# wangyunpeng139/3_ORB_SLAM3_SelfNote

Measured on AMD Instinct MI355X. Metric: frames/sec ORB extract+match, 752x480, higher is better.
Workload: dtype u8; 1 GPU; BASELINE configs[2]: extract + SearchByProjection match, 1000x1000 candidates, synthetic frame stream; image=752x480, nfeatures=1000, nlevels=8, batch=256, distinct_frames_per_gpu=2048, streams=4

## Files before the change

3_orb_slam3_selfnote_amd/csrc/orb_fast_score.h:

```cpp
#pragma once
#include <hip/hip_runtime.h>
#include <stdint.h>
#include "orb_common.h"

typedef short pk16 __attribute__((ext_vector_type(2)));

__host__ __device__ __forceinline__ int fast_score_S(const uint8_t *c ) {
  constexpr int Pt = FAST_TILE_PITCH;
  const int v = c[0];
  const pk16 V2 = {(short)v, (short)-v};
  const pk16 K = {(short)-1, (short)1};
  pk16 d[16];
#define ORB_RING(k, off) { const short cc = (short)c[off]; const pk16 C = {cc, cc}; d[k] = C * K + V2; }
  ORB_RING(0, 3 * Pt + 0)   ORB_RING(1, 3 * Pt + 1)   ORB_RING(2, 2 * Pt + 2)    ORB_RING(3, 1 * Pt + 3)
  ORB_RING(4, 3)            ORB_RING(5, -1 * Pt + 3)  ORB_RING(6, -2 * Pt + 2)   ORB_RING(7, -3 * Pt + 1)
  ORB_RING(8, -3 * Pt)      ORB_RING(9, -3 * Pt - 1)  ORB_RING(10, -2 * Pt - 2)  ORB_RING(11, -1 * Pt - 3)
  ORB_RING(12, -3)          ORB_RING(13, 1 * Pt - 3)  ORB_RING(14, 2 * Pt - 2)   ORB_RING(15, 3 * Pt - 1)
#undef ORB_RING
  pk16 m2[8], m4[8];
#pragma unroll
  for (int i = 0; i < 8; i++) m2[i] = __builtin_elementwise_min(d[2 * i + 1], d[(2 * i + 2) & 15]);
#pragma unroll
  for (int i = 0; i < 8; i++) m4[i] = __builtin_elementwise_min(m2[i], m2[(i + 1) & 7]);
  pk16 A;
#pragma unroll
  for (int i = 0; i < 8; i++) {
    const pk16 m8 = __builtin_elementwise_min(m4[i], m4[(i + 2) & 7]);
    const pk16 e = __builtin_elementwise_max(d[2 * i], d[(2 * i + 9) & 15]);
    const pk16 p = __builtin_elementwise_min(m8, e);
    A = i == 0 ? p : __builtin_elementwise_max(A, p);
  }
  const int a = A.x, b = A.y;
  const int S = a > b ? a : b;
  return S < 0 ? 0 : (S > 255 ? 255 : S);
}
```

3_orb_slam3_selfnote_amd/csrc/orb_kernels.h:

```cpp
#pragma once
#include <hip/hip_runtime.h>
#include <type_traits>
#include "orb_common.h"
#include "orb_fast_score.h"
#include "orb_sincos.h"

#define WAVE 64

__constant__ __attribute__((aligned(16))) int8_t c_pattern[1024] = {
#include "../../include/orb_pattern_data.inc"
};

struct DiscTab { uint32_t w[64][6]; };
constexpr DiscTab make_disc_tab() {
  DiscTab t{};
  const int umax[16] = {15, 15, 15, 15, 14, 14, 14, 13, 13, 12, 11, 10, 9, 8, 6, 3};
  int n = 0;
  for (int v = -15; v <= 15; v++) {
    const int d = umax[v < 0 ? -v : v];
    for (int u = -d; u <= d; u++) {
      const int lane = n & 63, k = n >> 6;
      t.w[lane][k >> 2] |= (uint32_t)(uint8_t)(int8_t)u << (8 * (k & 3));
      t.w[lane][3 + (k >> 2)] |= (uint32_t)(uint8_t)(int8_t)v << (8 * (k & 3));
      n++;
    }
  }
  return t;
}
__constant__ __attribute__((aligned(16))) DiscTab c_disc = make_disc_tab();

__device__ __forceinline__ int reflect101(int p, int n) {
  if (n == 1) return 0;
  while (p < 0 || p >= n) p = p < 0 ? -p : 2 * (n - 1) - p;
  return p;
}

__device__ __forceinline__ const uint8_t *level_plane(const FrameParams &P, int frame, int level, int &pitch) {
  if (level == 0) {
    pitch = (int)P.img0_stride;
    return P.img0 + (size_t)frame * P.img0_frame_stride;
  }
  pitch = P.geom[level].pitch;
  return P.pyr + (size_t)frame * P.pyr_fs + P.geom[level].off;
}

__device__ __forceinline__ void xcd_map(int nitems, uint32_t magic, int nframes, int &frame, int &item) {
  const unsigned b = blockIdx.x;
  const unsigned full = (unsigned)(nframes & ~7);
  const unsigned nfull = full * (unsigned)nitems;
  const bool inFull = b < nfull;
  const unsigned q = inFull ? (b >> 3) : (b - nfull);
  unsigned g = __umulhi(q, magic);
  unsigned r = q - g * (unsigned)nitems;
  if (r >= (unsigned)nitems) { g++; r -= (unsigned)nitems; }
  frame = (int)(inFull ? (b & 7u) + 8u * g : full + g);
  item = (int)r;
}

template <int CTRL, int ROWMASK>
__device__ __forceinline__ int dpp_or_zero(int v) { return __builtin_amdgcn_update_dpp(0, v, CTRL, ROWMASK, 0xf, false); }
__device__ __forceinline__ uint32_t mul24(uint32_t a, uint32_t u) {
  uint32_t d;
  asm("v_mul_u32_u24 %0, %1, %2" : "=v"(d) : "s"(u), "v"(a));
  return d;
}
__device__ __forceinline__ uint32_t mul24_vv(uint32_t a, uint32_t b) { return __umul24(a, b); }

__device__ __forceinline__ int wave_sum_i32(int v) {
  v += dpp_or_zero<0x111, 0xf>(v);
  v += dpp_or_zero<0x112, 0xf>(v);
  v += dpp_or_zero<0x114, 0xf>(v);
  v += dpp_or_zero<0x118, 0xf>(v);
  v += dpp_or_zero<0x142, 0xa>(v);
  v += dpp_or_zero<0x143, 0xc>(v);
  return __builtin_amdgcn_readlane(v, 63);
}

__device__ __forceinline__ uint32_t wave_incl_scan(uint32_t x) {
  int v = (int)x;
  v += dpp_or_zero<0x111, 0xf>(v);
  v += dpp_or_zero<0x112, 0xf>(v);
  v += dpp_or_zero<0x114, 0xf>(v);
  v += dpp_or_zero<0x118, 0xf>(v);
  v += dpp_or_zero<0x142, 0xa>(v);
  v += dpp_or_zero<0x143, 0xc>(v);
  return (uint32_t)v;
}

template <int NT>
__device__ uint32_t lds_excl_scan(uint32_t *a, int n, uint32_t *sw) {
  const int tid = threadIdx.x, lane = tid & 63, wid = tid >> 6;
  constexpr int NW = NT / 64;
  uint32_t carry = 0;
  for (int base = 0; base < n; base += NT) {
    int i = base + tid;
    uint32_t v = i < n ? a[i] : 0u;
    uint32_t inc = wave_incl_scan(v);
    if (lane == 63) sw[wid] = inc;
    __syncthreads();
    const uint32_t wsum = lane < NW ? sw[lane] : 0u;
    const uint32_t wincl = wave_incl_scan(wsum);
    const int widu = __builtin_amdgcn_readfirstlane(wid);
    const uint32_t woff = (uint32_t)__builtin_amdgcn_readlane((int)(wincl - wsum), widu);
    const uint32_t tot = (uint32_t)__builtin_amdgcn_readlane((int)wincl, NW - 1);
    if (i < n) a[i] = carry + woff + inc - v;
    carry += tot;
    __syncthreads();
  }
  return carry;
}

#define RESIZE_ROWS_MAX 16
#define RESIZE_MAXSRC 32
__global__ __launch_bounds__(256) void k_resize(FrameParams P, int level, int smemRowBytes, int tPitch, int maxSrc) {
  extern __shared__ __align__(16) uint8_t smem_rs[];
  const LevelGeom G = P.geom[level];
  const LevelGeom Gs = P.geom[level - 1];
  const int tid = threadIdx.x;
  int frame, rowTile;
  xcd_map((G.h + G.resizeRows - 1) / G.resizeRows, G.rowTileMagic, P.nframes, frame, rowTile);
  const int dy0 = rowTile * G.resizeRows;
  const int nrows = min(G.resizeRows, G.h - dy0);
  int spitch;
  const uint8_t *src = level_plane(P, frame, level - 1, spitch);
  uint8_t *dstplane = P.pyr + (size_t)frame * P.pyr_fs + G.off;
  const int wq = (G.w + 3) & ~3, qw = wq >> 2;
  __shared__ int2 sY[RESIZE_ROWS_MAX];
  if (tid < nrows) sY[tid] = P.ytab[G.ytabBase + dy0 + tid];

  if (tPitch > 0) {
    const int syFirst = min(max(P.ytab[G.ytabBase + dy0].x, 0), Gs.h - 1);
    const int syLast = min(max(P.ytab[G.ytabBase + dy0 + nrows - 1].x + 1, 0), Gs.h - 1);
    const int nsrc = min(syLast - syFirst + 1, maxSrc);
    uint8_t *sRows = smem_rs;
    uint8_t *sT = sRows + (size_t)maxSrc * smemRowBytes;
    uint4 *sRowRec = reinterpret_cast<uint4 *>(sT + (((size_t)maxSrc * tPitch + 15) & ~(size_t)15));
    const int4 *xtab4 = reinterpret_cast<const int4 *>(P.xtab + G.xtabBase);
    int4 xtPre[2];
#pragma unroll
    for (int k = 0; k < 2; k++) { const int p = tid + 256 * k; xtPre[k] = 2 * p < wq ? xtab4[p] : make_int4(0, 0, 0, 0); }
    const bool aligned = ((((uintptr_t)src) | (uintptr_t)spitch) & 3u) == 0;
    const uint8_t *src0 = src + (size_t)syFirst * spitch;
    if (aligned) {
      const int cpr = smemRowBytes >> 4, nfull = Gs.w >> 4;
      const float inv_cpr = 1.0f / (float)cpr;
      for (int idx = tid; idx < cpr * nsrc; idx += 256) {
        const int r = (int)(((float)idx + 0.5f) * inv_cpr), c = idx - (int)mul24((uint32_t)r, (uint32_t)cpr);
        if (c < nfull)
          __builtin_amdgcn_global_load_lds((const __attribute__((address_space(1))) void *)(src0 + (mul24((uint32_t)r, (uint32_t)spitch) + 16u * (uint32_t)c)),
                                           (__attribute__((address_space(3))) void *)(sRows + (size_t)(idx - (tid & 63)) * 16), 16, 0, 0);
      }
      const int ndw = (Gs.w + 3) >> 2, d0 = 4 * nfull, ntail = ndw - d0;
      const bool lastRowPartial = (Gs.w & 3) != 0;
      for (int idx = tid; idx < ntail * nsrc; idx += 256) {
        const int r = idx / ntail, d = d0 + (idx - r * ntail);
        const uint8_t *rowp = src0 + mul24((uint32_t)r, (uint32_t)spitch);
        uint32_t v;
        if (lastRowPartial && d == ndw - 1 && syFirst + r == Gs.h - 1 && spitch < 4 * ndw) {
          v = 0;
          for (int b = 0; 4 * d + b < Gs.w; b++) v |= (uint32_t)rowp[4 * d + b] << (8 * b);
        } else {
          v = *reinterpret_cast<const uint32_t *>(rowp + 4 * d);
        }
        *reinterpret_cast<uint32_t *>(sRows + mul24((uint32_t)r, (uint32_t)smemRowBytes) + 4 * d) = v;
      }
    } else {
      const float inv_w = 1.0f / (float)Gs.w;
      for (int idx = tid; idx < Gs.w * nsrc; idx += 256) {
        const int r = (int)(((float)idx + 0.5f) * inv_w), c = idx - (int)mul24((uint32_t)r, (uint32_t)Gs.w);
        sRows[mul24((uint32_t)r, (uint32_t)smemRowBytes) + c] = src0[mul24((uint32_t)r, (uint32_t)spitch) + c];
      }
    }
    if (tid < nrows) {
      const int2 yt = P.ytab[G.ytabBase + dy0 + tid];
      const int sy0 = min(max(yt.x, 0), Gs.h - 1), sy1 = min(max(yt.x + 1, 0), Gs.h - 1);
      sRowRec[tid] = make_uint4((uint32_t)((sy0 - syFirst) * tPitch), (uint32_t)((sy1 - syFirst) * tPitch), (uint32_t)yt.y, (uint32_t)((dy0 + tid) * G.pitch));
    }
    __syncthreads();
    typedef unsigned short u16x2 __attribute__((ext_vector_type(2)));
    auto dot2 = [](uint32_t pix, uint32_t coef) -> uint32_t {
      u16x2 x, y;
      __builtin_memcpy(&x, &pix, 4); __builtin_memcpy(&y, &coef, 4);
// ... 934 lines not shown
    for (int t = 0; t < 2; t++) {
      const uint32_t idx = (uint32_t)(lane + 64 * t), r = (idx * 21846u) >> 16, c = idx - 3u * r;
      if (idx < 111u)
        __builtin_amdgcn_global_load_lds((const __attribute__((address_space(1))) void *)(brow + (mul24(r, (uint32_t)G.bpitch) + 16u * c)),
                                         (__attribute__((address_space(3))) void *)&myPatch[idx * 16], 16, 0, 0);
    }
  }
  int m10 = 0, m01 = 0;
  int dv[12], du[12], dval[12];
  {
    const uint32_t uw[3] = {dw0.x, dw0.y, dw0.z}, vw[3] = {dw0.w, dw1.x, dw1.y};
#pragma unroll
    for (int t = 0; t < 12; t++) {
      du[t] = (int)(int8_t)(uw[t >> 2] >> (8 * (t & 3)));
      dv[t] = (int)(int8_t)(vw[t >> 2] >> (8 * (t & 3)));
    }
  }
  __shared__ __align__(16) uint8_t sDisc[4][31 * 48];
  uint8_t *myDisc = sDisc[threadIdx.x >> 6];
  if (((((uintptr_t)img) | (uintptr_t)pitch) & 3u) == 0) {
    const int qx0 = (X - 15) & ~3, qox = (X - 15) - qx0;
    const uint8_t *irow = img + (size_t)(Y - 15) * pitch + qx0;
#pragma unroll
    for (int t = 0; t < 2; t++) {
      const uint32_t idx = (uint32_t)(lane + 64 * t), r = (idx * 21846u) >> 16, c = idx - 3u * r;
      if (idx < 93u)
        __builtin_amdgcn_global_load_lds((const __attribute__((address_space(1))) void *)(irow + (mul24(r, (uint32_t)pitch) + 16u * c)),
                                         (__attribute__((address_space(3))) void *)&myDisc[idx * 16], 16, 0, 0);
    }
    asm volatile("s_waitcnt vmcnt(0)" ::: "memory");
    const uint8_t *dc = myDisc + 15 * 48 + qox + 15;
#pragma unroll
    for (int t = 0; t < 12; t++) dval[t] = dc[dv[t] * 48 + du[t]];
  } else {
#pragma unroll
    for (int t = 0; t < 12; t++) dval[t] = centre[dv[t] * pitch + du[t]];
  }
#pragma unroll
  for (int t = 0; t < 12; t++) { m10 += du[t] * dval[t]; m01 += dv[t] * dval[t]; }
  m10 = wave_sum_i32(m10);
  m01 = wave_sum_i32(m01);
  const float angle = fast_atan2_deg((float)m01, (float)m10);

  const float factorPI = (float)(3.1415926535897932384626433832795 / 180.f);
  const float arad = angle * factorPI;
  const float a = orbsc::ref_cosf(arad), b = orbsc::ref_sinf(arad);
  const uint8_t *bc = myPatch + 18 * 48 + pox + 18;
  constexpr int bp = 48;
  unsigned long long bits[4];
  int o0[4], o1[4];
#pragma unroll
  for (int r = 0; r < 4; r++) {
    const float x0 = (float)(int8_t)(pw[r] & 0xff), y0 = (float)(int8_t)((pw[r] >> 8) & 0xff);
    const float x1 = (float)(int8_t)((pw[r] >> 16) & 0xff), y1 = (float)(int8_t)(pw[r] >> 24);
    o0[r] = __float2int_rn(x0 * b + y0 * a) * bp + __float2int_rn(x0 * a - y0 * b);
    o1[r] = __float2int_rn(x1 * b + y1 * a) * bp + __float2int_rn(x1 * a - y1 * b);
  }
  asm volatile("s_waitcnt vmcnt(0)" ::: "memory");
  int v0[4], v1[4];
#pragma unroll
  for (int r = 0; r < 4; r++) { v0[r] = bc[o0[r]]; v1[r] = bc[o1[r]]; }
#pragma unroll
  for (int r = 0; r < 4; r++) bits[r] = __ballot(v0[r] < v1[r]);
  if (dst < P.cap) {
    uint32_t *dd = reinterpret_cast<uint32_t *>(P.out_desc + ((size_t)frame * P.cap + dst) * 32);
    if (lane < 8) {
      unsigned long long w = bits[lane >> 1];
      dd[lane] = (uint32_t)((lane & 1) ? (w >> 32) : w);
    }
    if (lane == 8) {
      KpOut k;
      k.x = (float)X;
      k.y = (float)Y;
      if (level != 0) { k.x = k.x * G.scale; k.y = k.y * G.scale; }
      k.size = G.kpsize;
      k.angle = angle;
      k.response = (float)(packed >> 24);
      k.octave = level;
      k.class_id = -1;
      reinterpret_cast<KpOut *>(P.out_kps)[(size_t)frame * P.cap + dst] = k;
    }
  }
}

template <int LANEBIT>
__device__ __forceinline__ int tr_step(int a, int b, int lane) {
  constexpr int CTRL = LANEBIT == 3 ? 0x140 : LANEBIT == 2 ? 0x141 : LANEBIT == 1 ? 0x4e : 0xb1;
  const bool hi = ((lane >> LANEBIT) & 1) != 0;
  const int keep = hi ? b : a, give = hi ? a : b;
  return keep + dpp_or_zero<CTRL, 0xf>(give);
}
template <int LOG, int LO, int N, class F>
__device__ __forceinline__ void tr_range(F &one, int lane, int &r10, int &r01) {
  if constexpr (N == 1) one(std::integral_constant<int, LO>{}, r10, r01);
  else {
    int a10, a01, b10, b01;
    tr_range<LOG, LO, N / 2>(one, lane, a10, a01);
    tr_range<LOG, LO + N / 2, N / 2>(one, lane, b10, b01);
    constexpr int S = N == 2 ? 0 : N == 4 ? 1 : N == 8 ? 2 : 3;
    r10 = tr_step<LOG - 1 - S>(a10, b10, lane);
    r01 = tr_step<LOG - 1 - S>(a01, b01, lane);
  }
}

typedef const __attribute__((address_space(3))) uint8_t *LdsBytes;
typedef const __attribute__((address_space(1))) uint8_t *GlobalBytes;
#define DESC_BUF (37 * 48)
#define DESC_WAVE_LDS (2 * DESC_BUF + 512)

template <int K>
__device__ __forceinline__ void describe_block(const FrameParams &P) {
  static_assert(K == 4 || K == 8 || K == 16, "a block is a quad, a half row or a row of DPP lanes");
  constexpr int LOG = K == 16 ? 4 : K == 8 ? 3 : 2;
  const int lane = threadIdx.x & 63;
  const int wid = __builtin_amdgcn_readfirstlane((int)(threadIdx.x >> 6));
  int frame, wg;
  xcd_map(ORB_DESCRIBE_GROUPS(P.totalKp, K), P.magicKpBlk, P.nframes, frame, wg);
  const int j0 = (wg * 4 + wid) * K;
  if (j0 >= P.totalKp) return;
  __shared__ __align__(16) uint8_t sDesc[4][DESC_WAVE_LDS];
  uint8_t *myLds = sDesc[wid];

  int cL = 0, lpL = 0, kbL = 0;
  if (lane < P.nlevels) {
    const int2 v = reinterpret_cast<const int2 *>(P.lcnt + (size_t)frame * P.nlevels * 2)[lane];
    cL = v.x; lpL = v.y;
    kbL = P.geom[lane].kpBase;
  }
  const int j = j0 + lane;
  int level = 0, kb = __builtin_amdgcn_readlane(kbL, 0), myCount = __builtin_amdgcn_readlane(cL, 0);
  int lapBefore = 0, monoBefore = 0, nTot = myCount, lapTot = __builtin_amdgcn_readlane(lpL, 0);
  for (int l = 1; l < P.nlevels; l++) {
    const int c = __builtin_amdgcn_readlane(cL, l), lp = __builtin_amdgcn_readlane(lpL, l), base = __builtin_amdgcn_readlane(kbL, l);
    const bool ge = j >= base;
    level = ge ? l : level; kb = ge ? base : kb; myCount = ge ? c : myCount;
    lapBefore = ge ? lapTot : lapBefore; monoBefore = ge ? nTot - lapTot : monoBefore;
    nTot += c; lapTot += lp;
  }
  if (j0 == 0 && lane == 0) { P.out_counts[frame * 2] = nTot; P.out_counts[frame * 2 + 1] = nTot - lapTot; }
  const bool valid = lane < K && j < P.totalKp && j - kb < myCount;
  const uint32_t validMask = (uint32_t)__ballot(valid);
  if (validMask == 0) return;
  uint32_t packed = 0, rk = 0;
  if (valid) { packed = P.lkp[(size_t)frame * P.lkp_fs + j]; rk = P.lrank[(size_t)frame * P.lkp_fs + j]; }
  const int X = (int)(packed & 0xfff) + ORB_MIN_BORDER, Y = (int)((packed >> 12) & 0xfff) + ORB_MIN_BORDER;
  const int dst = (rk & 0x8000u) ? nTot - 1 - (lapBefore + (int)(rk & 0x7fff)) : monoBefore + (int)(rk & 0x7fff);
  int pitch = (int)P.img0_stride;
  const uint8_t *img = P.img0 + (size_t)frame * P.img0_frame_stride;
  if (level != 0) { pitch = P.geom[level].pitch; img = P.pyr + (size_t)frame * P.pyr_fs + P.geom[level].off; }
  const uint8_t *centre = img + (size_t)Y * pitch + X;
  const uint32_t dmaMask = (uint32_t)__ballot(valid && ((((uintptr_t)img) | (uintptr_t)pitch) & 3u) == 0);
  const uint32_t cenLo = (uint32_t)(uintptr_t)centre, cenHi = (uint32_t)((uintptr_t)centre >> 32);

  const uint4 dw0 = *reinterpret_cast<const uint4 *>(&c_disc.w[lane][0]);
  const uint2 dw1 = *reinterpret_cast<const uint2 *>(&c_disc.w[lane][4]);
  const uint32_t uw[3] = {dw0.x, dw0.y, dw0.z}, vw[3] = {dw0.w, dw1.x, dw1.y};
  uint32_t doff2[6];
#pragma unroll
  for (int t = 0; t < 12; t += 2) {
    auto place = [&](int tt) { return (uint32_t)((int)(int8_t)(vw[tt >> 2] >> (8 * (tt & 3))) * 48 + (int)(int8_t)(uw[tt >> 2] >> (8 * (tt & 3))) + 15 * 48 + 15); };
    doff2[t >> 1] = place(t) | (place(t + 1) << 16);
    asm volatile("" : "+v"(doff2[t >> 1]));
  }
  const uint32_t cr0 = ((uint32_t)lane * 21846u) >> 16, cc0 = 16u * ((uint32_t)lane - 3u * cr0);
  const uint32_t cr1 = ((uint32_t)(lane + 64) * 21846u) >> 16, cc1 = 16u * ((uint32_t)(lane + 64) - 3u * cr1);
  auto issue = [&](const uint8_t *row0, uint32_t rowPitch, int which, uint32_t nchunks) {
    uint8_t *buf = myLds + which * DESC_BUF;
    asm volatile("s_waitcnt lgkmcnt(0)" ::: "memory");
    __builtin_amdgcn_global_load_lds((const __attribute__((address_space(1))) void *)(row0 + (mul24(cr0, rowPitch) + cc0)),
                                     (__attribute__((address_space(3))) void *)&buf[lane * 16], 16, 0, 0);
    if ((uint32_t)lane + 64u < nchunks)
      __builtin_amdgcn_global_load_lds((const __attribute__((address_space(1))) void *)(row0 + (mul24(cr1, rowPitch) + cc1)),
                                       (__attribute__((address_space(3))) void *)&buf[(lane + 64) * 16], 16, 0, 0);
  };
  auto centre_of = [&](uint32_t lo, uint32_t hi, int k) {
    return (uintptr_t)(uint32_t)__builtin_amdgcn_readlane((int)lo, k) | ((uintptr_t)(uint32_t)__builtin_amdgcn_readlane((int)hi, k) << 32);
  };
  auto issue_disc = [&](int k) {
    const uintptr_t c15 = centre_of(cenLo, cenHi, k) - 15;
    const uint32_t p = (uint32_t)__builtin_amdgcn_readlane(pitch, k);
    issue(reinterpret_cast<const uint8_t *>(c15 & ~(uintptr_t)3) - 15 * (size_t)p, p, k & 1, 93u);
  };

  if (dmaMask & 1u) issue_disc(0);
  auto one = [&](auto kc, int &p10, int &p01) {
    constexpr int k = decltype(kc)::value;
    const bool nextDma = k + 1 < K && ((dmaMask >> ((k + 1) & 31)) & 1u) != 0;
    if (nextDma) issue_disc(k + 1);
    p10 = 0; p01 = 0;
    if ((validMask >> k) & 1u) {
      uint32_t dval[12], dpk[3];
      const uintptr_t cen = centre_of(cenLo, cenHi, k);
      if ((dmaMask >> k) & 1u) {
        if (nextDma) asm volatile("s_waitcnt vmcnt(2)" ::: "memory");
        else asm volatile("s_waitcnt vmcnt(0)" ::: "memory");
        const LdsBytes dc = (LdsBytes)(myLds + (k & 1) * DESC_BUF + ((cen - 15) & 3));
#pragma unroll
        for (int t = 0; t < 12; t++) dval[t] = dc[(t & 1) ? doff2[t >> 1] >> 16 : doff2[t >> 1] & 0xffffu];
#pragma unroll
        for (int g = 0; g < 3; g++) dpk[g] = (dval[4 * g] | (dval[4 * g + 1] << 8)) | ((dval[4 * g + 2] | (dval[4 * g + 3] << 8)) << 16);
      } else {
        const GlobalBytes cp = (GlobalBytes)cen;
        const int p = __builtin_amdgcn_readlane(pitch, k);
        uint32_t uo[3], vo[3];
#pragma unroll
        for (int g = 0; g < 3; g++) { uo[g] = uw[g]; vo[g] = vw[g]; asm volatile("" : "+v"(uo[g]), "+v"(vo[g])); }
#pragma unroll
        for (int t = 0; t < 12; t++)
          dval[t] = cp[(int)(int8_t)(vo[t >> 2] >> (8 * (t & 3))) * p + (int)(int8_t)(uo[t >> 2] >> (8 * (t & 3)))];
#pragma unroll
        for (int g = 0; g < 3; g++) dpk[g] = (dval[4 * g] | (dval[4 * g + 1] << 8)) | ((dval[4 * g + 2] | (dval[4 * g + 3] << 8)) << 16);
      }
#pragma unroll
      for (int g = 0; g < 3; g++) {
        const uint32_t d = dpk[g] ^ 0x80808080u;
        p10 = __builtin_amdgcn_sdot4((int)uw[g], (int)d, p10, false);
        p01 = __builtin_amdgcn_sdot4((int)vw[g], (int)d, p01, false);
      }
    }
  };
  int r10, r01;
  tr_range<LOG, 0, K>(one, lane, r10, r01);
  int2 *sRed = reinterpret_cast<int2 *>(myLds + 2 * DESC_BUF);
  sRed[lane] = make_int2(r10, r01);
  int m10 = 0, m01 = 0;
  if (lane < K) {
    const int q = (int)(__builtin_bitreverse32((uint32_t)lane) >> (32 - LOG));
#pragma unroll
    for (int g = 0; g < 64 / K; g++) { const int2 v = sRed[q + K * g]; m10 += v.x; m01 += v.y; }
  }
  const int bpitch = P.geom[level].bpitch;
  const uint8_t *bcentre = P.blur + (size_t)frame * P.blur_fs + P.geom[level].boff + (size_t)Y * bpitch + X;
  const uint32_t bcenLo = (uint32_t)(uintptr_t)bcentre, bcenHi = (uint32_t)((uintptr_t)bcentre >> 32);
  auto issue_patch = [&](int k, int which) {
    const uintptr_t c18 = centre_of(bcenLo, bcenHi, k) - 18;
    const uint32_t p = (uint32_t)__builtin_amdgcn_readlane(bpitch, k);
    issue(reinterpret_cast<const uint8_t *>(c18 & ~(uintptr_t)3) - 18 * (size_t)p, p, which, 111u);
  };
  issue_patch(__builtin_ctz(validMask), 0);

  const float angle = fast_atan2_deg((float)m01, (float)m10);
  const float factorPI = (float)(3.1415926535897932384626433832795 / 180.f);
  const float arad = angle * factorPI;
  const float ca = orbsc::ref_cosf(arad), sb = orbsc::ref_sinf(arad);

  float pf[16];
#pragma unroll
  for (int r = 0; r < 4; r++) {
    const uint32_t pw = reinterpret_cast<const uint32_t *>(c_pattern)[r * 64 + lane];
    pf[4 * r] = (float)(int8_t)(pw & 0xff); pf[4 * r + 1] = (float)(int8_t)((pw >> 8) & 0xff);
    pf[4 * r + 2] = (float)(int8_t)((pw >> 16) & 0xff); pf[4 * r + 3] = (float)(int8_t)(pw >> 24);
  }
  constexpr int bp = 48;
  int which = 0;
  for (uint32_t m = validMask; m != 0; which ^= 1) {
    const int k = __builtin_ctz(m);
    m &= m - 1;
    if (m != 0) issue_patch(__builtin_ctz(m), which ^ 1);
    const float a = __builtin_bit_cast(float, __builtin_amdgcn_readlane(__builtin_bit_cast(int, ca), k));
    const float b = __builtin_bit_cast(float, __builtin_amdgcn_readlane(__builtin_bit_cast(int, sb), k));
    auto rn_bits = [](float v) { return __float_as_uint(v + 12582912.0f); };
    constexpr uint32_t RN_BIAS = 48u * 0x400000u + 0x4b400000u;
    uint32_t o0[4], o1[4];
#pragma unroll
    for (int r = 0; r < 4; r++) {
      const float x0 = pf[4 * r], y0 = pf[4 * r + 1], x1 = pf[4 * r + 2], y1 = pf[4 * r + 3];
      o0[r] = __umul24(rn_bits(x0 * b + y0 * a), (uint32_t)bp) + rn_bits(x0 * a - y0 * b);
      o1[r] = __umul24(rn_bits(x1 * b + y1 * a), (uint32_t)bp) + rn_bits(x1 * a - y1 * b);
    }
    if (m != 0) asm volatile("s_waitcnt vmcnt(2)" ::: "memory");
    else asm volatile("s_waitcnt vmcnt(0)" ::: "memory");
    const uint32_t bc = (uint32_t)(uintptr_t)(LdsBytes)myLds + (uint32_t)(which * DESC_BUF + 18 * 48 + 18) + (uint32_t)((centre_of(bcenLo, bcenHi, k) - 18) & 3) - RN_BIAS;
    int v0[4], v1[4];
#pragma unroll
    for (int r = 0; r < 4; r++) { v0[r] = *(LdsBytes)(uintptr_t)(bc + o0[r]); v1[r] = *(LdsBytes)(uintptr_t)(bc + o1[r]); }
    unsigned long long bits[4];
#pragma unroll
    for (int r = 0; r < 4; r++) bits[r] = __ballot(v0[r] < v1[r]);
    const int d = __builtin_amdgcn_readlane(dst, k);
    if (d < P.cap && lane < 8) {
      const unsigned long long w = bits[lane >> 1];
      reinterpret_cast<uint32_t *>(P.out_desc + ((size_t)frame * P.cap + d) * 32)[lane] = (uint32_t)((lane & 1) ? (w >> 32) : w);
    }
  }
  if (valid && dst < P.cap) {
    KpOut o;
    o.x = (float)X;
    o.y = (float)Y;
    if (level != 0) { const float sc = P.geom[level].scale; o.x = o.x * sc; o.y = o.y * sc; }
    o.size = P.geom[level].kpsize;
    o.angle = angle;
    o.response = (float)(packed >> 24);
    o.octave = level;
    o.class_id = -1;
    reinterpret_cast<KpOut *>(P.out_kps)[(size_t)frame * P.cap + dst] = o;
  }
}

template <int K>
__global__ __launch_bounds__(256, K == 1 ? 1 : 8) void k_describe(FrameParams P) {
  if constexpr (K == 1) describe_one(P);
  else describe_block<K>(P);
}

__global__ __launch_bounds__(256) void k_cvt_gray(const uint8_t *src, int rows, int cols, size_t sstride, int ch, int rgb, uint8_t *dst,
                                                  size_t dstride) {
  const int q = blockIdx.x * 256 + threadIdx.x, y = blockIdx.y;
  const int x0 = 4 * q;
  if (x0 >= cols || y >= rows) return;
  const uint8_t *s = src + (size_t)y * sstride + (size_t)x0 * ch;
  const int cr = rgb ? 0 : 2, cb = rgb ? 2 : 0;
  uint32_t packed = 0;
  const int n = min(4, cols - x0);
  for (int j = 0; j < n; j++) {
    const uint32_t g = ((uint32_t)s[j * ch + cr] * 4899u + (uint32_t)s[j * ch + 1] * 9617u + (uint32_t)s[j * ch + cb] * 1868u + 8192u) >> 14;
    packed |= g << (8 * j);
  }
  uint8_t *d = dst + (size_t)y * dstride + x0;
  if (n == 4 && ((((uintptr_t)dst) | dstride) & 3u) == 0) *reinterpret_cast<uint32_t *>(d) = packed;
  else for (int j = 0; j < n; j++) d[j] = (uint8_t)(packed >> (8 * j));
}

__device__ __forceinline__ uint8_t clahe_lut_entry(int v, int t, int clipLimit, float lutScale, uint32_t *hist, int *part) {
  if (clipLimit > 0) {
    int excess = v > clipLimit ? v - clipLimit : 0;
    if (v > clipLimit) v = clipLimit;
    const int ws = wave_sum_i32(excess);
    if ((t & 63) == 0) part[t >> 6] = ws;
    __syncthreads();
    const int clipped = part[0] + part[1] + part[2] + part[3];
    const int redistBatch = clipped / 256;
    const int residual = clipped - redistBatch * 256;
    v += redistBatch;
    if (residual != 0) {
      const int step = max(256 / residual, 1);
      if (t % step == 0 && t / step < residual) v++;
    }
  }
  __syncthreads();
  hist[t] = (uint32_t)v;
  __syncthreads();
  for (int d = 1; d < 256; d <<= 1) {
    const uint32_t a = t >= d ? hist[t - d] : 0u;
    __syncthreads();
    hist[t] += a;
    __syncthreads();
  }
  const int r = __float2int_rn(__fmul_rn((float)(int)hist[t], lutScale));
  return (uint8_t)min(max(r, 0), 255);
}

__global__ __launch_bounds__(256) void k_clahe_lut(const uint8_t *src, int rows, int cols, size_t sstride, int tilesX, int tw, int th, int clipLimit,
                                                   float lutScale, uint8_t *lut) {
  __shared__ uint32_t hist[256];
  __shared__ int part[4];
  const int t = threadIdx.x, tile = blockIdx.x, tx = tile % tilesX, ty = tile / tilesX;
  hist[t] = 0;
  __syncthreads();
  const int x0 = tx * tw, y0 = ty * th;
  for (int i = t; i < tw * th; i += 256) {
    int y = y0 + i / tw, x = x0 + i % tw;
    if (y >= rows) y = 2 * (rows - 1) - y;
    if (x >= cols) x = 2 * (cols - 1) - x;
    atomicAdd(&hist[src[(size_t)y * sstride + x]], 1u);
  }
  __syncthreads();
  lut[(size_t)tile * 256 + t] = clahe_lut_entry((int)hist[t], t, clipLimit, lutScale, hist, part);
}

__host__ __device__ __forceinline__ void clahe_tile_coord(int v, float inv_t, int ntiles, int &t1, int &t2, float &a, float &a1) {
// ... 257 lines not shown
```

Measured before the change: 296,600 frames/s.

## Use row-major disc layout with vector LDS reads and packed-half min3/max3 FAST score

The orientation moment loop now assigns each lane half of one disc row. It reads 20 contiguous bytes from LDS with a b128 plus b32 load, aligns them with alignbyte, and applies masked u/v weight words. This replaces 12 scattered byte LDS reads per lane. The FAST score biases its values to be positive so packed fp16 minimum/maximum can act as 3-input min/max on the integer bit patterns, and it reduces the final max as a tree to shorten the dependency chain. The change adds one extra sdot group and relies on the fp16 ordering trick, which is only correct while the biased values stay positive.

```diff
diff --git a/3_orb_slam3_selfnote_amd/csrc/orb_fast_score.h b/3_orb_slam3_selfnote_amd/csrc/orb_fast_score.h
--- a/3_orb_slam3_selfnote_amd/csrc/orb_fast_score.h
+++ b/3_orb_slam3_selfnote_amd/csrc/orb_fast_score.h
@@ -5,10 +5,30 @@
 
 typedef short pk16 __attribute__((ext_vector_type(2)));
 
+constexpr int FAST_BIAS = 2048;
+__host__ __device__ __forceinline__ pk16 fast_min3(pk16 a, pk16 b, pk16 c) {
+#if defined(__HIP_DEVICE_COMPILE__)
+  typedef _Float16 pkh __attribute__((ext_vector_type(2)));
+  return __builtin_bit_cast(pk16, __builtin_elementwise_minimum(__builtin_elementwise_minimum(__builtin_bit_cast(pkh, a), __builtin_bit_cast(pkh, b)),
+                                                                __builtin_bit_cast(pkh, c)));
+#else
+  return __builtin_elementwise_min(__builtin_elementwise_min(a, b), c);
+#endif
+}
+__host__ __device__ __forceinline__ pk16 fast_max3(pk16 a, pk16 b, pk16 c) {
+#if defined(__HIP_DEVICE_COMPILE__)
+  typedef _Float16 pkh __attribute__((ext_vector_type(2)));
+  return __builtin_bit_cast(pk16, __builtin_elementwise_maximum(__builtin_elementwise_maximum(__builtin_bit_cast(pkh, a), __builtin_bit_cast(pkh, b)),
+                                                                __builtin_bit_cast(pkh, c)));
+#else
+  return __builtin_elementwise_max(__builtin_elementwise_max(a, b), c);
+#endif
+}
+
 __host__ __device__ __forceinline__ int fast_score_S(const uint8_t *c ) {
   constexpr int Pt = FAST_TILE_PITCH;
   const int v = c[0];
-  const pk16 V2 = {(short)v, (short)-v};
+  const pk16 V2 = {(short)(FAST_BIAS + v), (short)(FAST_BIAS - v)};
   const pk16 K = {(short)-1, (short)1};
   pk16 d[16];
 #define ORB_RING(k, off) { const short cc = (short)c[off]; const pk16 C = {cc, cc}; d[k] = C * K + V2; }
@@ -17,20 +37,18 @@
   ORB_RING(8, -3 * Pt)      ORB_RING(9, -3 * Pt - 1)  ORB_RING(10, -2 * Pt - 2)  ORB_RING(11, -1 * Pt - 3)
   ORB_RING(12, -3)          ORB_RING(13, 1 * Pt - 3)  ORB_RING(14, 2 * Pt - 2)   ORB_RING(15, 3 * Pt - 1)
 #undef ORB_RING
-  pk16 m2[8], m4[8];
+  pk16 m2[8], m4[8], p[8];
 #pragma unroll
   for (int i = 0; i < 8; i++) m2[i] = __builtin_elementwise_min(d[2 * i + 1], d[(2 * i + 2) & 15]);
 #pragma unroll
   for (int i = 0; i < 8; i++) m4[i] = __builtin_elementwise_min(m2[i], m2[(i + 1) & 7]);
-  pk16 A;
 #pragma unroll
   for (int i = 0; i < 8; i++) {
-    const pk16 m8 = __builtin_elementwise_min(m4[i], m4[(i + 2) & 7]);
     const pk16 e = __builtin_elementwise_max(d[2 * i], d[(2 * i + 9) & 15]);
-    const pk16 p = __builtin_elementwise_min(m8, e);
-    A = i == 0 ? p : __builtin_elementwise_max(A, p);
+    p[i] = fast_min3(m4[i], m4[(i + 2) & 7], e);
   }
-  const int a = A.x, b = A.y;
+  const pk16 A = __builtin_elementwise_max(fast_max3(p[0], p[1], p[2]), fast_max3(fast_max3(p[3], p[4], p[5]), p[6], p[7]));
+  const int a = A.x - FAST_BIAS, b = A.y - FAST_BIAS;
   const int S = a > b ? a : b;
   return S < 0 ? 0 : (S > 255 ? 255 : S);
 }
diff --git a/3_orb_slam3_selfnote_amd/csrc/orb_kernels.h b/3_orb_slam3_selfnote_amd/csrc/orb_kernels.h
--- a/3_orb_slam3_selfnote_amd/csrc/orb_kernels.h
+++ b/3_orb_slam3_selfnote_amd/csrc/orb_kernels.h
@@ -12,12 +12,12 @@
 };
 
 struct DiscTab { uint32_t w[64][6]; };
+constexpr int kDiscUmax[16] = {15, 15, 15, 15, 14, 14, 14, 13, 13, 12, 11, 10, 9, 8, 6, 3};
 constexpr DiscTab make_disc_tab() {
   DiscTab t{};
-  const int umax[16] = {15, 15, 15, 15, 14, 14, 14, 13, 13, 12, 11, 10, 9, 8, 6, 3};
   int n = 0;
   for (int v = -15; v <= 15; v++) {
-    const int d = umax[v < 0 ? -v : v];
+    const int d = kDiscUmax[v < 0 ? -v : v];
     for (int u = -d; u <= d; u++) {
       const int lane = n & 63, k = n >> 6;
       t.w[lane][k >> 2] |= (uint32_t)(uint8_t)(int8_t)u << (8 * (k & 3));
@@ -28,6 +28,11 @@
   return t;
 }
 __constant__ __attribute__((aligned(16))) DiscTab c_disc = make_disc_tab();
+constexpr uint64_t make_disc_umax_nibbles() {
+  uint64_t p = 0;
+  for (int v = 0; v < 16; v++) p |= (uint64_t)kDiscUmax[v] << (4 * v);
+  return p;
+}
 
 __device__ __forceinline__ int reflect101(int p, int n) {
   if (n == 1) return 0;
@@ -1268,15 +1273,22 @@
   const uint32_t dmaMask = (uint32_t)__ballot(valid && ((((uintptr_t)img) | (uintptr_t)pitch) & 3u) == 0);
   const uint32_t cenLo = (uint32_t)(uintptr_t)centre, cenHi = (uint32_t)((uintptr_t)centre >> 32);
 
-  const uint4 dw0 = *reinterpret_cast<const uint4 *>(&c_disc.w[lane][0]);
-  const uint2 dw1 = *reinterpret_cast<const uint2 *>(&c_disc.w[lane][4]);
-  const uint32_t uw[3] = {dw0.x, dw0.y, dw0.z}, vw[3] = {dw0.w, dw1.x, dw1.y};
-  uint32_t doff2[6];
-#pragma unroll
-  for (int t = 0; t < 12; t += 2) {
-    auto place = [&](int tt) { return (uint32_t)((int)(int8_t)(vw[tt >> 2] >> (8 * (tt & 3))) * 48 + (int)(int8_t)(uw[tt >> 2] >> (8 * (tt & 3))) + 15 * 48 + 15); };
-    doff2[t >> 1] = place(t) | (place(t + 1) << 16);
-    asm volatile("" : "+v"(doff2[t >> 1]));
+  const int drow = min(lane >> 1, 30), dhalf = lane & 1, dvv = drow - 15;
+  const uint32_t rowOff = (uint32_t)(drow * 48 + 16 * dhalf);
+  uint32_t wu[4], wv[4];
+  {
+    const int d = (int)((make_disc_umax_nibbles() >> (4 * (dvv < 0 ? -dvv : dvv))) & 15u);
+    const int first = dhalf ? 0 : 15 - d, end = lane < 62 ? (dhalf ? d : 16) : first;
+    const uint32_t vrep = (uint32_t)(dvv & 0xff) * 0x01010101u;
+#pragma unroll
+    for (int i = 0; i < 4; i++) {
+      const int lo = min(max(first - 4 * i, 0), 4), hi = min(max(end - 4 * i, 0), 4);
+      const uint32_t inside = (uint32_t)(0xffffffffull << (8 * lo)) & ~(uint32_t)(0xffffffffull << (8 * hi));
+      auto ub = [](int u0) { return (uint32_t)(uint8_t)u0 | ((uint32_t)(uint8_t)(u0 + 1) << 8) | ((uint32_t)(uint8_t)(u0 + 2) << 16) | ((uint32_t)(uint8_t)(u0 + 3) << 24); };
+      wu[i] = (dhalf ? ub(4 * i + 1) : ub(4 * i - 15)) & inside;
+      wv[i] = vrep & inside;
+      asm volatile("" : "+v"(wu[i]), "+v"(wv[i]));
+    }
   }
   const uint32_t cr0 = ((uint32_t)lane * 21846u) >> 16, cc0 = 16u * ((uint32_t)lane - 3u * cr0);
   const uint32_t cr1 = ((uint32_t)(lane + 64) * 21846u) >> 16, cc1 = 16u * ((uint32_t)(lane + 64) - 3u * cr1);
@@ -1305,33 +1317,42 @@
     if (nextDma) issue_disc(k + 1);
     p10 = 0; p01 = 0;
     if ((validMask >> k) & 1u) {
-      uint32_t dval[12], dpk[3];
       const uintptr_t cen = centre_of(cenLo, cenHi, k);
       if ((dmaMask >> k) & 1u) {
         if (nextDma) asm volatile("s_waitcnt vmcnt(2)" ::: "memory");
         else asm volatile("s_waitcnt vmcnt(0)" ::: "memory");
-        const LdsBytes dc = (LdsBytes)(myLds + (k & 1) * DESC_BUF + ((cen - 15) & 3));
-#pragma unroll
-        for (int t = 0; t < 12; t++) dval[t] = dc[(t & 1) ? doff2[t >> 1] >> 16 : doff2[t >> 1] & 0xffffu];
-#pragma unroll
-        for (int g = 0; g < 3; g++) dpk[g] = (dval[4 * g] | (dval[4 * g + 1] << 8)) | ((dval[4 * g + 2] | (dval[4 * g + 3] << 8)) << 16);
+        const uint32_t rp = (uint32_t)(uintptr_t)(LdsBytes)myLds + rowOff;
+        typedef uint32_t u32x4 __attribute__((ext_vector_type(4)));
+        u32x4 q;
+        uint32_t q4;
+        asm volatile("ds_read_b128 %0, %2 offset:%3\n\tds_read_b32 %1, %2 offset:%4\n\ts_waitcnt lgkmcnt(0)"
+                     : "=&v"(q), "=&v"(q4) : "v"(rp), "n"((k & 1) * DESC_BUF), "n"((k & 1) * DESC_BUF + 16) : "memory");
+        const uint32_t raw[5] = {q.x, q.y, q.z, q.w, q4};
+        const uint32_t o = (uint32_t)((cen - 15) & 3);
+#pragma unroll
+        for (int g = 0; g < 4; g++) {
+          const uint32_t d = __builtin_amdgcn_alignbyte(raw[g + 1], raw[g], o) ^ 0x80808080u;
+          p10 = __builtin_amdgcn_sdot4((int)wu[g], (int)d, p10, false);
+          p01 = __builtin_amdgcn_sdot4((int)wv[g], (int)d, p01, false);
+        }
       } else {
-        const GlobalBytes cp = (GlobalBytes)cen;
-        const int p = __builtin_amdgcn_readlane(pitch, k);
-        uint32_t uo[3], vo[3];
-#pragma unroll
-        for (int g = 0; g < 3; g++) { uo[g] = uw[g]; vo[g] = vw[g]; asm volatile("" : "+v"(uo[g]), "+v"(vo[g])); }
+        const uint32_t p = (uint32_t)__builtin_amdgcn_readlane(pitch, k);
+        const GlobalBytes cp = (GlobalBytes)cen - (15 * (size_t)p + 15);
+        int tl = lane;
+        asm volatile("" : "+v"(tl));
+        const uint4 dw0 = *reinterpret_cast<const uint4 *>(&c_disc.w[tl][0]);
+        const uint2 dw1 = *reinterpret_cast<const uint2 *>(&c_disc.w[tl][4]);
+        const uint32_t uw[3] = {dw0.x, dw0.y, dw0.z}, vw[3] = {dw0.w, dw1.x, dw1.y};
+        uint32_t dval[12];
 #pragma unroll
         for (int t = 0; t < 12; t++)
-          dval[t] = cp[(int)(int8_t)(vo[t >> 2] >> (8 * (t & 3))) * p + (int)(int8_t)(uo[t >> 2] >> (8 * (t & 3)))];
-#pragma unroll
-        for (int g = 0; g < 3; g++) dpk[g] = (dval[4 * g] | (dval[4 * g + 1] << 8)) | ((dval[4 * g + 2] | (dval[4 * g + 3] << 8)) << 16);
-      }
-#pragma unroll
-      for (int g = 0; g < 3; g++) {
-        const uint32_t d = dpk[g] ^ 0x80808080u;
-        p10 = __builtin_amdgcn_sdot4((int)uw[g], (int)d, p10, false);
-        p01 = __builtin_amdgcn_sdot4((int)vw[g], (int)d, p01, false);
+          dval[t] = cp[(uint32_t)((int)(int8_t)(vw[t >> 2] >> (8 * (t & 3))) + 15) * p + (uint32_t)((int)(int8_t)(uw[t >> 2] >> (8 * (t & 3))) + 15)];
+#pragma unroll
+        for (int g = 0; g < 3; g++) {
+          const uint32_t d = ((dval[4 * g] | (dval[4 * g + 1] << 8)) | ((dval[4 * g + 2] | (dval[4 * g + 3] << 8)) << 16)) ^ 0x80808080u;
+          p10 = __builtin_amdgcn_sdot4((int)uw[g], (int)d, p10, false);
+          p01 = __builtin_amdgcn_sdot4((int)vw[g], (int)d, p01, false);
+        }
       }
     }
   };
```

Measured after the change: 300,300 frames/s, median of 6. 1.01x the previous value.
